# lpastura/kubernetes-1

Measured on AMD Instinct MI355X. Metric: pods scheduled/sec, higher is better.
Workload: dtype int64; 1 GPU; (b) 5000 nodes / 1913000 pods; nodes=5000, nodes_per_gpu=5000, pods=1913000, percentage_of_nodes_to_score=100, parallelism=1 GPU

## Files before the change

include/kgpu.h:

```cpp
#ifndef KGPU_H
#define KGPU_H

#include <stdint.h>

#ifdef __cplusplus
extern "C" {
#endif

#define KGPU_ABI_VERSION 3

#define KGPU_OK 0
#define KGPU_E_INVAL (-1)
#define KGPU_E_NOMEM (-2)
#define KGPU_E_DEVICE (-3)
#define KGPU_E_CAPACITY (-4)
#define KGPU_E_STATE (-5)
#define KGPU_E_UNSUPPORTED (-6)

#define KGPU_CODE_SUCCESS 0
#define KGPU_CODE_ERROR 1
#define KGPU_CODE_UNSCHEDULABLE 2
#define KGPU_CODE_UNRESOLVABLE 3

#define KGPU_F_NODE_UNSCHEDULABLE 0
// ... 383 lines not shown
#define KGPU_OPT_PERSISTENT 2
#define KGPU_OPT_PERSIST_GROUPS 3
#define KGPU_OPT_PHASE_TRACE 4
#define KGPU_OPT_TOPO_FUSED 5
#define KGPU_OPT_TOPO_PERSISTENT 6
#define KGPU_OPT_ABORT_AT 7
#define KGPU_OPT_XGMI 8
#define KGPU_OPT_SKIP_RELEASE_AT 9
#define KGPU_OPT_COOPERATIVE 10
#define KGPU_OPT_BATCH_GEO 11
#define KGPU_OPT_ARENA_BYTES 12
#define KGPU_OPT_TOPO_RESIDENT 13
#define KGPU_OPT_BATCH_HELPER 14
#define KGPU_OPT_TOPO_AHEAD 15
#define KGPU_OPT_TBATCH_GEO 16
#define KGPU_OPT_HOLD_GROUP 17
#define KGPU_OPT_TBATCH_WLAB 18
#define KGPU_OPT_RUN_ALL_FILTERS 20
#define KGPU_OPT_TBATCH_POLL_SLEEP 21
#define KGPU_OPT_ZEROCOPY_POOLS 23
#define KGPU_OPT_CUT_PERSISTENT 24
#define KGPU_OPT_CUT_TOPO_PERSISTENT 25
#define KGPU_OPT_NORM_PERSISTENT 26
int kgpu_set_option(kgpu_ctx* ctx, int32_t option, int64_t value);
int kgpu_debug_counters(const kgpu_ctx* ctx, int64_t* out, int32_t n);
int kgpu_geometry_for(int32_t kernel, int32_t n_nodes, int32_t max_groups, int32_t first, int32_t out[4]);
int kgpu_debug_geometry(const kgpu_ctx* ctx, int32_t out[6]);
int kgpu_debug_instantiation(const kgpu_ctx* ctx, int32_t out[4]);
int kgpu_debug_topo_resident(const kgpu_ctx* ctx, int64_t out[2]);
int kgpu_read_phase_trace(kgpu_ctx* ctx, int64_t* out, int32_t max_iters);

typedef struct kgpu_nominated {
  int32_t node;
  int32_t item;
} kgpu_nominated;
int kgpu_set_nominated(kgpu_ctx* ctx, const kgpu_nominated* noms, int32_t n, const kgpu_pod_query* pods,
                       const kgpu_pools* pools);

typedef struct kgpu_victim {
  int32_t node;
  int32_t slot;
  int32_t item;
  int32_t pad;
  int64_t start_time;
  uint64_t pdb_mask;
} kgpu_victim;
// ... 56 lines not shown
```

kubernetes-1_amd/csrc/kgpu_api.cpp:

```cpp
#include <hip/hip_runtime.h>
#include <rccl/rccl.h>
#include <dlfcn.h>
#include <execinfo.h>
#include <fcntl.h>
#include <signal.h>
#include <unistd.h>

#include <algorithm>
#include <array>
#include <chrono>
#include <atomic>
#include <exception>
#include <memory>
#include <new>
#include <iterator>
#include <cmath>
#include <cstdio>
#include <cstdlib>
#include <cstddef>
#include <cstring>
#include <deque>
#include <map>
#include <string>
#include <unordered_map>
// ... 139 lines not shown
  void* res_pin = nullptr;
  kgpu_result* res_dev = nullptr;
  void* pool_pin = nullptr;
  const char* pool_pin_dev = nullptr;
  bool zc_pools = true;
  kgpu::Arena ar;
  bool tb_abort_mapped = false;
  struct TCache {
    bool valid = false;
    std::string key;
    DevBuf buf[2];
    size_t dirty[2] = {0, 0};
    int cur = 0;
  } tc;
  uint64_t tc_hits = 0, tc_misses = 0;
  bool htrace = false;
  static constexpr int kHt = 18;
  int64_t ht_last = 0, ht_cur[kHt] = {}, ht_n = 0;
  int ht_seen = 0;
  std::vector<std::array<int64_t, kHt>> ht_cycles;
  std::vector<std::array<int64_t, kHt>> ht_batches;
  bool tc_on = true;
  bool batch_helper = true;
  bool topo_ahead = true;
  int tbatch_geo_first = 1;
  size_t ar_limit = 1 << 20;
  DevState ds_last{};
  const void* ds_ptr = nullptr;
  bool last_diag = false;
  std::vector<int64_t> trace_wg_host;
  int32_t trace_wg_groups = 0;
  std::vector<hipEvent_t> ev_pool;
  std::map<std::vector<int64_t>, int> class_ids, tclass_ids;
  std::vector<kgpu::ClassRec> classes;
  std::vector<kgpu::ClassItem> citems;
  std::vector<kgpu::TermClassRec> tclasses;
  std::vector<kgpu_req> creqs;
  std::vector<int32_t> cints;
  int classes_init = 0;
  int Ccap = 0, TCcap = 0;
  DevBuf d_classes, d_citems, d_tclasses, d_creqs, d_cints, d_plans, d_aux, d_aux_terms, scratch, d_pods;
  struct PodRow {
    int32_t node, ns;
    uint32_t flags;
    std::vector<int32_t> pairs;
    std::vector<int32_t> own_tcls;
// ... 2040 lines not shown
      if (cut) {
        const size_t cells = (size_t)cnt * 2 * (size_t)groups;
        const size_t gbytes = (sizeof(uint64_t) * (cells + (size_t)cnt) + 15) & ~(size_t)15;
        if ((rc = ensure(c, c->cgran, gbytes))) return rc;
        HIP_OK(c, hipMemsetAsync(c->cgran.p, 0, gbytes, c->stream));
        ba.cgran = static_cast<uint64_t*>(c->cgran.p);
        ba.cpos = ba.cgran + cells;
        ba.cut_nofilt = c->cfg.n_filters == 0 ? 1 : 0;
        ba.nranks = 1;
        ba.GT = groups;
      } else if (xg) {
        const size_t cells = (size_t)kgpu::kXgmiRing * (size_t)c->xg_GT;
        ba.gran = static_cast<uint64_t*>(c->xg_box.p);
        ba.feas = reinterpret_cast<int32_t*>(ba.gran + cells);
        ba.pgran = static_cast<uint64_t* const*>(c->xg_arr.p);
        ba.pfeas = reinterpret_cast<int32_t* const*>(static_cast<uint64_t* const*>(c->xg_arr.p) + c->xg_nranks);
        ba.nranks = c->xg_nranks;
        ba.rank = c->xg_rank;
        ba.GT = c->xg_GT;
        ba.R = kgpu::kXgmiRing;
        ba.xseq0 = c->xg_seq;
        c->xg_seq += cnt;
      } else {
        const size_t cells = (size_t)cnt * (size_t)groups;
        const size_t gbytes = sizeof(uint64_t) * cells + sizeof(int32_t) * cells;
        if ((rc = ensure(c, c->gran, gbytes))) return rc;
        HIP_OK(c, hipMemsetAsync(c->gran.p, 0, sizeof(uint64_t) * cells, c->stream));
        ba.gran = static_cast<uint64_t*>(c->gran.p);
        ba.feas = reinterpret_cast<int32_t*>(ba.gran + cells);
        run_ptrs.push_back({ba.gran, ba.feas});
        void** slot = static_cast<void**>(c->batch_ptrs.p) + 2 * (run_ptrs.size() - 1);
        if ((rc = stage_h2d(c, slot, run_ptrs.back().data(), sizeof(void*) * 2))) return rc;
        ba.pgran = reinterpret_cast<uint64_t* const*>(slot);
        ba.pfeas = reinterpret_cast<int32_t* const*>(slot + 1);
        ba.nranks = 1;
        ba.rank = 0;
        ba.GT = groups;
        ba.R = 0;
      }
      ba.first = i;
      ba.count = cnt;
      ba.per = per;
      ba.assume = assume;
      ba.seq0 = first_seq + i;
      ba.abort = abort_word;
      ba.abort_at = c->abort_at >= i && c->abort_at < i + cnt ? c->abort_at - i : -1;
      ba.skip_release_at = c->skip_release_at >= i && c->skip_release_at < i + cnt ? c->skip_release_at - i : -1;
// ... 832 lines not shown
  int per = 0, groups = 0;
  const int kidx = kgpu::batch_geometry(c->st.N, std::min(c->max_groups > 0 ? std::min(c->max_groups, c->n_cus) : c->n_cus, 256),
                                        &per, &groups, c->batch_geo_first);
  if (kidx < 0) return fail(c, KGPU_E_UNSUPPORTED, "no persistent geometry for this node count");
  if ((rc = upload_pools(c, pools))) return rc;
  if (!c->ticket.p) {
    if ((rc = ensure(c, c->ticket, 9 * 64))) return rc;
    HIP_OK(c, hipMemset(c->ticket.p, 0, 9 * 64));
  }
  const int s = c->pipe_next;
  c->pipe_next ^= 1;
  kgpu_ctx::PipeSlot& ps = c->pipe[s];
  const size_t q_off = kDsQueryOff, q_bytes = sizeof(kgpu_pod_query) * (size_t)n;
  const size_t p_off = (q_off + q_bytes + 15) & ~(size_t)15, a_off = p_off + 16 * 2;
  const size_t bytes = a_off + 64;
  if ((rc = ensure(c, ps.dev, bytes))) return rc;
  if (ps.host_cap < bytes) {
    if (ps.host) HIP_OK(c, hipHostFree(ps.host));
    ps.host = nullptr;
    ps.host_cap = 0;
    HIP_OK(c, hipHostMalloc(&ps.host, bytes * 2, hipHostMallocDefault));
    ps.host_cap = bytes * 2;
  }
  const size_t cells = (size_t)n * (size_t)groups;
  const size_t gbytes = (sizeof(uint64_t) + sizeof(int32_t)) * cells;
  if (ps.gran.bytes < gbytes) {
    if ((rc = ensure(c, ps.gran, gbytes))) return rc;
    ps.gran_zeroed = 0;
  }
  if (ps.gran_zeroed < gbytes) {
    HIP_OK(c, hipMemsetAsync(ps.gran.p, 0, ps.gran.bytes, c->stream));
    ps.gran_zeroed = ps.gran.bytes;
  }
  const size_t rbytes = sizeof(kgpu_result) * (size_t)n + 64;
  if (ps.res_cap < rbytes) {
    if (ps.res) HIP_OK(c, hipHostFree(ps.res));
    ps.res = nullptr;
    ps.res_cap = 0;
    HIP_OK(c, hipHostMalloc(&ps.res, rbytes * 2, hipHostMallocCoherent | hipHostMallocMapped));
    HIP_OK(c, hipHostGetDevicePointer(&ps.res_dev, ps.res, 0));
    ps.res_cap = rbytes * 2;
  }
  for (hipEvent_t* e : {&ps.done, &ps.t0, &ps.t1})
    if (!*e) HIP_OK(c, hipEventCreateWithFlags(e, e == &ps.done ? hipEventDisableTiming : hipEventDefault));
  char* h = static_cast<char*>(ps.host);
  char* d = static_cast<char*>(ps.dev.p);
  DevState st = c->st;
// ... 1 lines not shown
  st.queries = reinterpret_cast<const kgpu_pod_query*>(d + q_off);
  if ((rc = ensure(c, c->results, sizeof(kgpu_result) * (size_t)n))) return rc;
  st.results = static_cast<kgpu_result*>(c->results.p);
  st.diag_raw = nullptr;
  st.diag_norm = nullptr;
  uint64_t* gran = static_cast<uint64_t*>(ps.gran.p);
  int32_t* feas = reinterpret_cast<int32_t*>(gran + cells);
  std::memcpy(h, &st, sizeof(DevState));
  std::memcpy(h + q_off, qs, q_bytes);
  void* ptrs[2] = {gran, feas};
  std::memcpy(h + p_off, ptrs, sizeof(ptrs));
  std::memset(h + a_off, 0, 64);
  HIP_OK(c, hipMemcpyAsync(d, h, bytes, hipMemcpyHostToDevice, c->stream));
  c->tc.valid = false;
  kgpu::BatchArgs ba{};
  ba.gran = gran;
  ba.feas = feas;
  ba.pgran = reinterpret_cast<uint64_t* const*>(d + p_off);
  ba.pfeas = reinterpret_cast<int32_t* const*>(d + p_off + sizeof(void*));
  ba.nranks = 1;
  ba.rank = 0;
  ba.GT = groups;
  ba.R = 0;
  ba.first = 0;
  ba.count = n;
  ba.per = per;
  ba.assume = 1;
  ba.seq0 = first_seq;
  ba.abort = reinterpret_cast<int32_t*>(d + a_off);
  ba.abort_at = -1;
  ba.skip_release_at = -1;
  ba.trace = nullptr;
  ba.res_out = static_cast<kgpu_result*>(ps.res_dev);
  ba.abort_out = reinterpret_cast<int32_t*>(static_cast<char*>(ps.res_dev) + sizeof(kgpu_result) * (size_t)n);
  kgpu_ctx::PipeSlot& po = c->pipe[s ^ 1];
  ba.zero_buf = static_cast<uint64_t*>(po.gran.p);
  ba.zero_n16 = po.gran.p ? (int64_t)(po.gran.bytes / 16) : 0;
  const bool coop = c->coop;
  ba.hold = -1;
  ++c->n_persist;
  c->n_coop += coop ? 1 : 0;
  *reinterpret_cast<int32_t*>(static_cast<char*>(ps.res) + sizeof(kgpu_result) * (size_t)n) = -1;
  const bool timed = stats != nullptr;
  if (timed) HIP_OK(c, hipEventRecord(ps.t0, c->stream));
  note_geometry(c, 1, kidx, groups, per);
  note_instantiation(c, kgpu::batch_row(c->spec), false, kgpu::batch_helper_used(c->spec, kidx, false, c->batch_helper), n);
// ... 172 lines not shown
      if (cfg->filters[j] == cfg->filters[i]) return KGPU_E_INVAL;
  }
  if (cfg->percentage_of_nodes_to_score < 0 || cfg->percentage_of_nodes_to_score > 100) return KGPU_E_INVAL;
  for (int i = 0; i < cfg->n_scores; ++i)
    if (cfg->scores[i] == KGPU_S_REQUESTED_TO_CAPACITY_RATIO) {
      if (cfg->n_rtcr < 0 || cfg->n_rtcr > 8 || cfg->n_shape < 1 || cfg->n_shape > 16) return KGPU_E_INVAL;
      for (int j = 1; j < cfg->n_shape; ++j)
        if (cfg->shape[j].utilization <= cfg->shape[j - 1].utilization) return KGPU_E_INVAL;
    }
  fail_point();
  std::unique_ptr<kgpu_ctx> holder(new kgpu_ctx());
  kgpu_ctx* c = holder.get();
  int ndev = 0;
  if (hipGetDeviceCount(&ndev) != hipSuccess || ndev <= 0) return KGPU_E_DEVICE;
  if (cfg->device < 0 || cfg->device >= ndev) return KGPU_E_INVAL;
  c->cfg = *cfg;
  c->device = cfg->device;
  if (hipSetDevice(c->device) != hipSuccess) return KGPU_E_DEVICE;
  {
    const char* e = std::getenv("KGPU_SYNC_SPIN");
    if (e && e[0] == '1') (void)hipSetDeviceFlags(hipDeviceScheduleSpin);
  }
  if (const char* e = std::getenv("KGPU_HOST_TRACE")) c->htrace = e[0] == '1';
  if (hipStreamCreateWithFlags(&c->stream, hipStreamNonBlocking) != hipSuccess)
    return KGPU_E_DEVICE;
  hipDeviceProp_t prop;
  if (hipGetDeviceProperties(&prop, c->device) != hipSuccess) {
    (void)hipStreamDestroy(c->stream);
    return KGPU_E_DEVICE;
  }
  c->n_cus = prop.multiProcessorCount;
  DevState& st = c->st;
  st.n_filters = cfg->n_filters;
  std::memcpy(st.filters, cfg->filters, sizeof(st.filters));
  st.n_scores = cfg->n_scores;
  std::memcpy(st.scores, cfg->scores, sizeof(st.scores));
  for (int i = 0; i < KGPU_NUM_SCORES; ++i) st.weights[i] = std::max<int64_t>(cfg->score_weights[i], 1);
  for (int i = 0; i < KGPU_NUM_SCORES; ++i) st.w_of[i] = 0;
  for (int i = 0; i < cfg->n_scores; ++i) st.w_of[cfg->scores[i]] = st.weights[i];
  st.n_least = cfg->n_least;
  st.n_most = cfg->n_most;
  std::memcpy(st.least, cfg->least, sizeof(st.least));
  std::memcpy(st.most, cfg->most, sizeof(st.most));
  st.least_wsum = st.most_wsum = 0;
  for (int i = 0; i < cfg->n_least; ++i) st.least_wsum += cfg->least[i].weight;
  for (int i = 0; i < cfg->n_most; ++i) st.most_wsum += cfg->most[i].weight;
// ... 183 lines not shown
  std::memcpy(out, c->trace_wg_host.data(), sizeof(int64_t) * n);
  *groups = c->trace_wg_groups;
  return (int)std::min<size_t>(n, INT32_MAX);
} catch (...) {
  return on_exception(c, false);
}

int kgpu_set_option(kgpu_ctx* c, int32_t option, int64_t value) try {
  if (c && !c->pipe_q.empty())
    return fail(c, KGPU_E_STATE, "pipelined batches in flight: complete them with kgpu_schedule_batch_wait first");
  if (!c) return KGPU_E_INVAL;
  if (option == KGPU_OPT_KERNEL_TIMING) c->timing = value != 0;
  else if (option == KGPU_OPT_PERSISTENT) c->persistent = value != 0;
  else if (option == KGPU_OPT_PERSIST_GROUPS) c->max_groups = (int)std::max<int64_t>(value, 0);
  else if (option == KGPU_OPT_PHASE_TRACE) {
    c->phase_trace = value != 0;
    c->phase_trace_mode = (int)std::min<int64_t>(std::max<int64_t>(value, 0), 3);
  }
  else if (option == KGPU_OPT_TOPO_FUSED) c->topo_fused = value != 0;
  else if (option == KGPU_OPT_TOPO_PERSISTENT) c->tfast = value != 0;
  else if (option == KGPU_OPT_COOPERATIVE) c->coop = value != 0;
  else if (option == KGPU_OPT_BATCH_GEO) c->batch_geo_first = (int)std::min<int64_t>(std::max<int64_t>(0, value), 6);
  else if (option == KGPU_OPT_BATCH_HELPER) c->batch_helper = value != 0;
  else if (option == KGPU_OPT_TOPO_AHEAD) c->topo_ahead = value != 0;
  else if (option == KGPU_OPT_TBATCH_GEO) c->tbatch_geo_first = (int)std::min<int64_t>(std::max<int64_t>(value, 0), 4);
  else if (option == KGPU_OPT_TOPO_RESIDENT) {
    c->tc_on = value != 0;
    c->tc.valid = false;
  } else if (option == KGPU_OPT_ARENA_BYTES) c->ar_limit = (size_t)std::min<int64_t>(std::max<int64_t>(0, value), (int64_t)kArenaBytes);
  else if (option == KGPU_OPT_ABORT_AT) c->abort_at = value < 0 || value > INT32_MAX ? -1 : (int32_t)value;
  else if (option == KGPU_OPT_XGMI) c->xgmi = value != 0;
  else if (option == KGPU_OPT_TBATCH_WLAB) c->tbatch_wlab = value != 0;
  else if (option == KGPU_OPT_TBATCH_POLL_SLEEP) c->tbatch_sleep = value != 0;
  else if (option == KGPU_OPT_ZEROCOPY_POOLS) c->zc_pools = value != 0;
  else if (option == KGPU_OPT_RUN_ALL_FILTERS) c->run_all = value != 0;
  else if (option == KGPU_OPT_HOLD_GROUP) c->hold_group = value < 0 || value > INT32_MAX ? -1 : (int32_t)value;
  else if (option == KGPU_OPT_CUT_PERSISTENT) c->cut_persistent = value != 0;
  else if (option == KGPU_OPT_CUT_TOPO_PERSISTENT) c->cut_topo_persistent = value != 0;
  else if (option == KGPU_OPT_NORM_PERSISTENT) c->norm_persistent = (int32_t)std::min<int64_t>(std::max<int64_t>(value, 0), INT32_MAX);
  else if (option == KGPU_OPT_SKIP_RELEASE_AT) c->skip_release_at = value < 0 || value > INT32_MAX ? -1 : (int32_t)value;
  else return KGPU_E_INVAL;
  return KGPU_OK;
} catch (...) {
  return on_exception(c, false);
}

// ... 1055 lines not shown
```

kubernetes-1_amd/csrc/kgpu_internal.h:

```cpp
#pragma once
#include <stdint.h>

#include "../../include/kgpu.h"

namespace kgpu {

constexpr int kBlock = 64;
constexpr int kMaxBlocks = 1024;
constexpr int kSelAnd = 0, kSelNothing = 1, kSelEmpty = 2;
constexpr uint64_t kMask40 = (1ull << 40) - 1;
constexpr int kMaxRanks = 64;

struct BlkStat {
  int32_t feasible;
  int32_t max_taint;
  int32_t max_na;
  int32_t pad;
};
struct BlkKey {
  uint64_t key;
  int32_t idx;
  int32_t feasible;
};

// ... 173 lines not shown
  int32_t diag;
  int32_t cut;
  int32_t zero_diag;
  int32_t resolve_self;
  int32_t q_inline;
  int64_t seq;
  int32_t* done_out;
  kgpu_pod_query q;
};

struct BatchArgs {
  int32_t first;
  int32_t count;
  int32_t per;
  int32_t assume;
  int64_t seq0;
  uint64_t* gran;
  int32_t* feas;
  int32_t* abort;
  int64_t* trace;
  int32_t abort_at;
  int32_t skip_release_at;
  int32_t hold;
  int32_t pad_h;
  kgpu_result* res_out;
  int32_t* abort_out;
  uint64_t* zero_buf;
  int64_t zero_n16;
  uint64_t* const* pgran;
  int32_t* const* pfeas;
  int32_t nranks, rank;
  int32_t GT;
  int32_t R;
  int64_t xseq0;
  uint64_t* cgran;
  uint64_t* cpos;
  int32_t cut_nofilt;
  int32_t pad_c;
};
constexpr int32_t kAbortDirty = 1, kAbortClean = 2;
constexpr int kXgmiRing = 4096;
constexpr int kXgmiMaxGT = 1024;

constexpr int kTMaxSoftWords = 8;
constexpr int kTMaxZones = 32;
constexpr int kTLdsBudget = 144 * 1024;
constexpr int kTCutBytes = 544;
// ... 241 lines not shown
```

kubernetes-1_amd/csrc/kgpu_kernels.hip:

```cpp
#include <hip/hip_runtime.h>

#include <algorithm>
#include <map>
#include <mutex>
#include <tuple>
#include <type_traits>

#include "kgpu_internal.h"

#if defined(__HIP_DEVICE_COMPILE__)
#define GAS __attribute__((address_space(1)))
#define CAS __attribute__((address_space(4)))
#else
#define GAS
#define CAS
#endif

namespace kgpu {

template <class T>
__device__ __forceinline__ GAS T* gp(T* p) {
  return (GAS T*)p;
}
template <class T>
// ... 1302 lines not shown
  }
  if (!__all(all)) return false;
  wave_argmax(k, gsel);
  wkey = k;
  wg = k ? gsel : -1;
  return true;
}
template <int NJ, bool SYS>
__device__ __forceinline__ bool poll_row(const uint64_t* row, int G, const int32_t* abort_word, uint64_t tmask,
                                         uint64_t expect, uint64_t& wkey, int& wg) {
  const uint64_t t0 = __builtin_amdgcn_s_memrealtime();
  Sweep<NJ> a = sweep<NJ, SYS>(row, G, abort_word, expect);
  for (;;) {
    const Sweep<NJ> b = sweep<NJ, SYS>(row, G, abort_word, expect);
    if (a.abort != 0) return false;
    if (row_done<NJ>(a, tmask, expect, wkey, wg)) return true;
    a = sweep<NJ, SYS>(row, G, abort_word, expect);
    if (b.abort != 0) return false;
    if (row_done<NJ>(b, tmask, expect, wkey, wg)) return true;
    if (__builtin_amdgcn_s_memrealtime() - t0 > kSpinTimeout) return false;
  }
}

struct HRow {
  int64_t ac, am, zc, zm;
  double ic, im;
};

constexpr int kQRing = 4;
constexpr int kQWords = (int)(sizeof(kgpu_pod_query) / 8);
static_assert(kQWords <= 64, "one query row per vector load");
typedef uint64_t __attribute__((may_alias)) qword_t;
struct NoQuery {};
__device__ __forceinline__ kgpu_pod_query ring_read(const kgpu_pod_query* ring, int k) {
  const kgpu_pod_query& s = ring[k & (kQRing - 1)];
  kgpu_pod_query q{};
  q.flags = s.flags;
  q.req[0] = s.req[0]; q.req[1] = s.req[1]; q.req[2] = s.req[2];
  q.nz[0] = s.nz[0]; q.nz[1] = s.nz[1];
  q.score_req[0] = s.score_req[0]; q.score_req[1] = s.score_req[1];
  q.scalars = s.scalars;
  q.ports = s.ports;
  return q;
}
__device__ __forceinline__ kgpu_pod_query ring_uniform(kgpu_pod_query q) {
  q.flags = __builtin_amdgcn_readfirstlane(q.flags);
  q.scalars.begin = __builtin_amdgcn_readfirstlane(q.scalars.begin);
  q.scalars.count = __builtin_amdgcn_readfirstlane(q.scalars.count);
  q.ports.begin = __builtin_amdgcn_readfirstlane(q.ports.begin);
  q.ports.count = __builtin_amdgcn_readfirstlane(q.ports.count);
  return q;
}

template <uint32_t FM, uint32_t SM, int K, int B, bool XG, bool HB = false, bool TR = false>
__global__ __launch_bounds__(B + 64 + (HB ? 2 * B : 0)) void k_batch(const DevState* __restrict__ stp, BatchArgs pa) {
  static_assert(!HB || (B == 64 && !XG &&
                       SM == ((1u << KGPU_S_BALANCED_ALLOCATION) | (1u << KGPU_S_LEAST_ALLOCATED) | kDefRes)),
                "the helper wave splits config (b)'s profile on the one-row-wave geometry");
  static_assert(HB || !TR, "only the helper-wave instantiation has a traced twin");
  const DevState& st = *stp;
  constexpr int W = B / 64;
  const int tid = threadIdx.x, wave = tid >> 6, lane = tid & 63;
  const int G = gridDim.x, g = blockIdx.x;
  if (g == pa.hold) return;
  const int lo = g * pa.per;
  const int GT = pa.GT, gme = pa.rank * G + g;
  constexpr bool xg = XG;
  const uint64_t tmask = xg ? (0xFull << 60) : kGValid;
  __shared__ BatchShared<B> sh;
  __shared__ int64_t sh_hk[HB ? 2 * 2 * K * B : 1];
  __shared__ int sh_hready[2];
  __shared__ std::conditional_t<HB, kgpu_pod_query, NoQuery> sh_q[HB ? kQRing : 1];
  __shared__ uint64_t* sh_peer_g[XG ? kMaxRanks : 1];
  __shared__ int32_t* sh_peer_f[XG ? kMaxRanks : 1];
  if constexpr (XG) {
    if (wave == W && lane < pa.nranks) {
      sh_peer_g[lane] = pa.pgran[lane];
      sh_peer_f[lane] = pa.pfeas[lane];
    }
  }
  if (tid == 0) {
    sh.bready = 0;
// ... 4 lines not shown
  if constexpr (HB) {
    if (wave == W && lane < kQWords)
      for (int k = 0; k < 3 && k < pa.count; ++k)
        reinterpret_cast<qword_t*>(&sh_q[k])[lane] = ((const GAS qword_t*)(st.queries + pa.first + k))[lane];
  }
  __syncthreads();
  auto ring_row = [&](int k) -> size_t { return xg ? (size_t)((pa.xseq0 + k) % pa.R) : (size_t)k; };
  auto ring_tag = [&](int k) -> uint64_t {
    return xg ? (kGValid | ((uint64_t)(((pa.xseq0 + k) / pa.R) & 7) << 60)) : kGValid;
  };
  auto publish = [&](int i, uint64_t key, int feas) {
    const size_t roff = ring_row(i) * GT + gme;
    const uint64_t gtag = ring_tag(i);
    if constexpr (!XG) {
      store_sc1(pa.gran + roff, gtag | key);
      pa.feas[roff] = feas;
    } else {
      for (int rk = 0; rk < pa.nranks; ++rk) {
        __hip_atomic_store(sh_peer_g[rk] + roff, gtag | key, __ATOMIC_RELAXED, __HIP_MEMORY_SCOPE_SYSTEM);
        __hip_atomic_store(sh_peer_f[rk] + roff, feas, __ATOMIC_RELAXED, __HIP_MEMORY_SCOPE_SYSTEM);
      }
    }
  };
  const bool tr = pa.trace && (g == 0 || g == G - 1);
  int64_t* trow = pa.trace ? pa.trace + (g == 0 ? 0 : 8) : nullptr;
  constexpr bool kStamps = !HB || TR;
#define KGPU_STAMP(i, k) \
  if (kStamps && tr && (tid == 0 || tid == B)) trow[(size_t)(i) * 16 + (k)] = (int64_t)__builtin_amdgcn_s_memrealtime()

  if constexpr (HB) {
    if (wave == W + 1 || wave == W + 2) {
      const int hw = wave - W - 1;
      HRow h[K];
#pragma unroll
      for (int j = 0; j < K; ++j) {
        const int n = lo + j * B + lane;
        h[j] = HRow{0, 0, 0, 0, 0.0, 0.0};
        if (!spare_slot(j, K, lane, B) && n < st.N) {
          h[j].ac = gp(st.alloc_cpu)[n];
          h[j].am = gp(st.alloc_mem)[n];
          h[j].zc = gp(st.nz_cpu)[n];
          h[j].zm = gp(st.nz_mem)[n];
          h[j].ic = (h[j].ac > 0 && h[j].ac < (1ll << 52)) ? 1.0 / (double)h[j].ac : 0.0;
          h[j].im = (h[j].am > 0 && h[j].am < (1ll << 52)) ? 1.0 / (double)h[j].am : 0.0;
        }
      }
// ... 55 lines not shown
        }
        rqp = rq;
        rq = ring_uniform(rqn);
        const bool slow = have_cur && won && pa.assume && !fast_b;
        int cn = -1;
        if (have_cur && !slow) {
          const Cand c = wg_combine<B>(sh, p, won && fast_b);
          cn = c.key ? c.idx : -1;
        }
        if (slow) {
          lds_wait(&sh.cready, i + 1, pa.abort);
          cand = sh.cslow[p];
        } else {
          cand = cn;
        }
        staged = have_cur && !slow && cand >= 0;
      }
      return;
    }
  }
  if (wave == W) {
    int cand = -1;
    bool staged = false;
    for (int i = 0; i <= pa.count; ++i) {
      const bool have_prev = i > 0, have_cur = i < pa.count;
      const int p = i & 1;
      if (i == pa.abort_at && g == 0 && lane == 0) __hip_atomic_store(pa.abort, 1, __ATOMIC_RELAXED, __HIP_MEMORY_SCOPE_AGENT);
      uint64_t qv = 0;
      if constexpr (HB) {
        if (i + 3 < pa.count && lane < kQWords) qv = ((const GAS qword_t*)(st.queries + pa.first + i + 3))[lane];
      } else if (i + 2 < pa.count) {
        const uint64_t v = lane < kQWords ? reinterpret_cast<const uint64_t*>(st.queries + pa.first + i + 2)[lane] : 0;
        asm volatile("" ::"v"(v));
      }
      bool qmem = false;
      if (have_prev) {
        if constexpr (HB) {
          const kgpu_pod_query& qq = sh_q[(i - 1) & (kQRing - 1)];
          qmem = __builtin_amdgcn_readfirstlane(qq.scalars.count | qq.ports.count) != 0;
        } else {
          const kgpu_pod_query* qq = st.queries + pa.first + i - 1;
          qmem = (cp(qq)->scalars.count | cp(qq)->ports.count) != 0;
        }
      }
      const bool fast_b = have_prev && cand >= 0 && staged && pa.assume && !qmem;
      uint64_t wkey = 0;
      int wg = -1;
      bool ok = true;
      if (have_prev) {
        const uint64_t* prow = pa.gran + ring_row(i - 1) * GT;
        const uint64_t expect = ring_tag(i - 1);
        if constexpr (!XG)
          ok = poll_row<4, false>(prow, GT, pa.abort, tmask, expect, wkey, wg);
        else if (GT <= 256)
          ok = poll_row<4, true>(prow, GT, pa.abort, tmask, expect, wkey, wg);
        else
          ok = poll_row<16, true>(prow, GT, pa.abort, tmask, expect, wkey, wg);
        KGPU_STAMP(i, 7);
      }
      const bool won = have_prev && wg == gme;
      const bool slow = have_cur && won && pa.assume && !fast_b;
      if (ok) {
        if (have_prev && lane == 0 && (xg ? g == 0 : (won || (wg < 0 && g == 0)))) {
          kgpu_result res;
          res.node = wg < 0 ? -1
                   : xg ? (int32_t)rank40_inv(pod_tie_key(st.seed, pa.seq0 + i - 1), wkey & kMask40, st.tie_mode)
                        : st.node_base + lo + cand;
          res.feasible = 0;
          res.evaluated = st.n_total;
          res.scored = 0;
          res.score = wg >= 0 ? (int64_t)(wkey >> 40) - 1 : 0;
          gp(st.results)[pa.first + i - 1] = res;
        }
      } else if (lane == 0) {
        __hip_atomic_fetch_or(pa.abort, (i <= 1 && !XG) ? kAbortClean : kAbortDirty, __ATOMIC_RELAXED,
                              __HIP_MEMORY_SCOPE_AGENT);
      }
      if (lane == 0 && have_prev) {
        sh.rwg[(i - 1) & 1] = wg;
        sh.rabort[(i - 1) & 1] = ok ? 0 : 1;
      }
      __syncthreads();
      if (!ok) break;
      int cn = -1;
      if (have_cur && !slow) {
        KGPU_STAMP(i, 6);
        const Cand c = wg_combine<B>(sh, p, won && fast_b);
        if (lane == 0) publish(i, c.key, c.feas);
        KGPU_STAMP(i, 3);
        cn = c.key ? c.idx : -1;
      }
      if constexpr (HB) {
        if (i + 3 < pa.count && lane < kQWords) reinterpret_cast<qword_t*>(&sh_q[(i + 3) & (kQRing - 1)])[lane] = qv;
      }
      if (slow) {
        lds_wait(&sh.cready, i + 1, pa.abort);
        cand = sh.cslow[p];
      } else {
        cand = cn;
      }
      staged = have_cur && !slow && cand >= 0;
    }
    return;
  }

  constexpr bool kStream = K > 4;
  constexpr int KR = kStream ? 1 : K;
  static_assert(!kStream || (W > 1 && !HB), "streamed rows: the candidate row travels through sh.brow");
  constexpr bool kRecip = (SM & kDefRes) != 0 && SM != kRuntime;
  NodeRes r[KR];
#pragma unroll
  for (int j = 0; j < KR; ++j) {
    const int n = lo + j * B + tid;
    r[j] = NodeRes{};
    if (!kStream && !spare_slot(j, K, tid, B) && n < st.N) r[j] = load_row<kRecip>(st, n);
  }
  __builtin_amdgcn_s_waitcnt(0);

  kgpu_pod_query qp{};
  kgpu_pod_query q = *cp(st.queries + pa.first);
  if constexpr (HB) q = ring_uniform(ring_read(sh_q, 0));
  int cand = -1;
  bool staged = false;
  for (int i = 0; i <= pa.count; ++i) {
    KGPU_STAMP(i, 0);
    std::conditional_t<HB, kgpu_pod_query, NoQuery> qraw{};
    if constexpr (HB) qraw = ring_read(sh_q, i + 1);
    const bool have_prev = i > 0;
    const bool have_cur = i < pa.count;
    const int p = i & 1;
    const bool fast_b = have_prev && cand >= 0 && staged && pa.assume && qp.scalars.count == 0 && qp.ports.count == 0;
    const int ob = cand >= 0 ? cand % B : -1, jb = cand >= 0 ? cand / B : -1;
    uint64_t keys[K];
    Cand own_a{0, -1, 0}, own_b{0, -1, 0};
    if (have_cur) {
      const uint64_t tk = pod_tie_key(st.seed, pa.seq0 + i);
      if (fast_b && wave == W - 1) {
        NodeRes t;
        if constexpr (W == 1) {
#pragma unroll
          for (int j = 0; j < K; ++j)
            if (j == jb) t = lane_row(r[j], ob);
        } else {
          lds_wait(&sh.bready, i, pa.abort);
          t = sh.brow[(i - 1) & 1];
        }
        assume_regs(qp, t);
        if (tid == B - 1) r[KR - 1] = t;
      }
      if constexpr (HB) {
        uint32_t fs[K];
        uint64_t rkj[K];
#pragma unroll
        for (int j = 0; j < K; ++j) {
          const bool spare = spare_slot(j, K, tid, B);
          const int n = spare ? lo + cand : lo + j * B + tid;
          fs[j] = (spare ? fast_b : n < st.N) ? run_filters<FM>(st, q, r[j], n) : 1u;
// ... 4 lines not shown
        lds_wait_ge(&sh_hready[1], i + 1, pa.abort);
#pragma unroll
        for (int j = 0; j < K; ++j) {
          const int64_t tot = sh_hk[((0 * 2 + p) * K + j) * B + tid] + sh_hk[((1 * 2 + p) * K + j) * B + tid];
          keys[j] = fs[j] ? 0 : (((uint64_t)(tot + 1) << 40) | rkj[j]);
        }
      } else {
#pragma unroll
        for (int j = 0; j < K; ++j) {
          const bool spare = spare_slot(j, K, tid, B);
          const int n = spare ? lo + cand : lo + j * B + tid;
          if constexpr (kStream) {
            const bool live = spare ? fast_b : n < st.N;
            NodeRes rj = r[0];
            if (!spare && live) rj = load_row<kRecip>(st, n);
            keys[j] = live ? node_key<FM, SM>(st, q, rj, n, tk) : 0;
          } else {
            keys[j] = (spare ? fast_b : n < st.N) ? node_key<FM, SM>(st, q, r[j], n, tk) : 0;
          }
        }
      }
      KGPU_STAMP(i, 5);
      wg_partials<K, B>(sh, p, keys, fast_b, ob, jb, cand, own_a, own_b);
    }
    KGPU_STAMP(i, 1);
    kgpu_pod_query qn{};
    if constexpr (!HB) {
      if (i + 1 < pa.count) qn = *cp(st.queries + pa.first + i + 1);
    }
    __syncthreads();
    KGPU_STAMP(i, 2);
    int wg = -1;
    if (have_prev) {
      const int s = (i - 1) & 1;
      if (sh.rabort[s]) break;
      wg = sh.rwg[s];
    }
    if constexpr (HB) {
      if (i + 1 < pa.count) qn = ring_uniform(qraw);
    }
    const bool won = have_prev && wg == gme;
    int cn = -1;
    if (have_cur) {
      if (won && pa.assume && !fast_b) {
        cn = -2;
      } else {
// ... 8 lines not shown
          if constexpr (kStream) {
            NodeRes t = load_res(st, lo + (j * B + tid));
            assume_row(st, qp, t, lo + (j * B + tid));
          } else {
            assume_row(st, qp, r[j], lo + (j * B + tid));
          }
          assume_counts(st, pa.first + i - 1, lo + (j * B + tid));
        }
    }
    const bool slow = cn == -2;
    if (slow) {
      if (wave == ob / 64) {
        if (tid == ob) {
          const uint64_t tk = pod_tie_key(st.seed, pa.seq0 + i);
#pragma unroll
          for (int j = 0; j < K; ++j)
            if (j == jb) {
              if constexpr (kStream) keys[j] = node_key<FM, SM>(st, q, load_row<kRecip>(st, lo + (j * B + tid)), lo + (j * B + tid), tk);
              else keys[j] = node_key<FM, SM>(st, q, r[j], lo + (j * B + tid), tk);
            }
        }
        const Cand c = wave_recombine<K, B>(sh, p, keys);
        if (lane == 0) {
          publish(i, c.key, c.feas);
          sh.cslow[p] = c.key ? c.idx : -1;
          lds_release(&sh.cready, i + 1);
        }
      }
      lds_wait(&sh.cready, i + 1, pa.abort);
      cand = sh.cslow[p];
    } else {
      cand = cn;
      if (W > 1 && cand >= 0 && tid == cand % B) {
#pragma unroll
        for (int j = 0; j < K; ++j)
          if (j == cand / B) {
            if constexpr (kStream) sh.brow[p] = load_row<kRecip>(st, lo + cand);
            else sh.brow[p] = r[j];
          }
        if (i != pa.skip_release_at) lds_release(&sh.bready, i + 1);
      }
    }
    staged = have_cur && !slow && cand >= 0;
    qp = q;
    q = qn;
    KGPU_STAMP(i, 4);
  }
#undef KGPU_STAMP
}

__global__ __launch_bounds__(256) void k_batch_fixup(const DevState* __restrict__ stp, BatchArgs pa, int G) {
  const DevState& st = *stp;
  const int lane = threadIdx.x & 63;
  const int i = blockIdx.x * 4 + (threadIdx.x >> 6);
  for (int64_t z = (int64_t)blockIdx.x * blockDim.x + threadIdx.x; z < pa.zero_n16; z += (int64_t)gridDim.x * blockDim.x) {
    uint4* zp = reinterpret_cast<uint4*>(pa.zero_buf) + z;
    *zp = uint4{0, 0, 0, 0};
  }
  if (pa.abort_out && blockIdx.x == 0 && threadIdx.x == 0)
    __hip_atomic_store(pa.abort_out, load_sc1(pa.abort), __ATOMIC_RELAXED, __HIP_MEMORY_SCOPE_SYSTEM);
  if (i >= pa.count) return;
  const size_t row = pa.R > 0 ? (size_t)((pa.xseq0 + i) % pa.R) : (size_t)i;
  int f = 0;
  for (int g = lane; g < pa.GT; g += 64) f += pa.feas[row * pa.GT + g];
  f = (int)wave_sum32((uint32_t)f);
  (void)G;
  if (lane == 0) {
    kgpu_result& r = gp(st.results)[pa.first + i];
    r.feasible = f;
    if (r.node >= 0 && f >= 2) {
      r.scored = 1;
    } else {
      r.scored = 0;
      r.score = 0;
    }
    if (pa.res_out) pa.res_out[pa.first + i] = r;
  }
}

template <int NJ>
__device__ __forceinline__ bool poll_counts(const uint64_t* row, int G, int g, const int32_t* abort_word,
                                            uint32_t (&out)[4]) {
  const int lane = threadIdx.x & 63;
  const uint64_t t0 = __builtin_amdgcn_s_memrealtime();
  for (;;) {
    const Sweep<NJ> a = sweep<NJ, false>(row, G, abort_word, kGValid);
    if (__any(a.abort != 0)) return false;
// ... 2731 lines not shown

struct Geo {
  int B, K;
};
constexpr Geo kGeo[] = {{64, 1}, {128, 1}, {192, 1}, {448, 1}, {960, 1}, {512, 4}, {512, 8}};
constexpr int kNumGeo = sizeof(kGeo) / sizeof(kGeo[0]);
constexpr int kBatchLdsPad = 96 * 1024;

template <uint32_t FM, uint32_t SM>
struct BatchRow {
  using Fn = void (*)(const DevState*, BatchArgs);
  static constexpr Fn fn[kNumGeo] = {k_batch<FM, SM, 1, 64, false>,  k_batch<FM, SM, 1, 128, false>,
                                     k_batch<FM, SM, 1, 192, false>, k_batch<FM, SM, 1, 448, false>,
                                     k_batch<FM, SM, 1, 960, false>, k_batch<FM, SM, 4, 512, false>,
                                     k_batch<FM, SM, 8, 512, false>};
  static constexpr Fn xfn[kNumGeo] = {k_batch<FM, SM, 1, 64, true>,  k_batch<FM, SM, 1, 128, true>,
                                      k_batch<FM, SM, 1, 192, true>, k_batch<FM, SM, 1, 448, true>,
                                      k_batch<FM, SM, 1, 960, true>, k_batch<FM, SM, 4, 512, true>,
                                      k_batch<FM, SM, 8, 512, true>};
};
using BatchFn = void (*)(const DevState*, BatchArgs);
template <uint32_t FM, uint32_t SM, bool E>
struct HelperFn {
  static constexpr BatchFn fn = nullptr, traced = nullptr;
};
template <uint32_t FM, uint32_t SM>
struct HelperFn<FM, SM, true> {
  static constexpr BatchFn fn = k_batch<FM, SM, 1, 64, false, true>;
  static constexpr BatchFn traced = k_batch<FM, SM, 1, 64, false, true, true>;
};
static const BatchFn kBatchHelper[] = {
    nullptr,
    HelperFn<kFitFM, kFitSM, true>::fn,
    nullptr,
    nullptr,
};
static const BatchFn kBatchHelperTraced[] = {
    nullptr,
    HelperFn<kFitFM, kFitSM, true>::traced,
    nullptr,
    nullptr,
};
static const BatchFn* const kBatch[] = {
    BatchRow<kRuntime, kRuntime>::fn,
    BatchRow<kFitFM, kFitSM>::fn,
    BatchRow<kDefaultFM, kDefaultSM>::fn,
    BatchRow<kDefaultFM, kAutoscalerSM>::fn,
};
static_assert(sizeof(kBatch) / sizeof(kBatch[0]) == kNumSpecs, "one k_batch row per profile instantiation");
static const BatchFn* const kBatchX[] = {
    BatchRow<kRuntime, kRuntime>::xfn,
    BatchRow<kFitFM, kFitSM>::xfn,
    BatchRow<kDefaultFM, kDefaultSM>::xfn,
    BatchRow<kDefaultFM, kAutoscalerSM>::xfn,
};

int batch_geometry(int N, int max_groups, int* per, int* groups, int first) {
  for (int gi = first < 0 ? 0 : first; gi < kNumGeo; ++gi) {
    const int p = kGeo[gi].B * kGeo[gi].K - 1;
    const int g = (N + p - 1) / p;
    if (g <= max_groups) {
      *per = p;
// ... 11 lines not shown
    return true;
  }
  if (kernel == 2 && geo >= 0 && geo < kNumTGeo) {
    *threads = kTGeo[geo].B;
    *rows = kTGeo[geo].K;
    return true;
  }
  return false;
}

int batch_row(int spec) { return spec < 0 || spec >= kNumSpecs ? 0 : spec; }

bool batch_helper_used(int spec, int geo, bool sharded, bool helper) {
  return helper && !sharded && geo == 0 && kBatchHelper[batch_row(spec)] != nullptr;
}

int launch_batch(const DevState* st, const BatchArgs& a, int groups, int geo, int spec, bool coop, bool helper,
                 void* stream) {
  spec = batch_row(spec);
  if (geo < 0 || geo >= kNumGeo) return -1;
  const int x = a.R > 0 ? 1 : 0;
  const bool hb = batch_helper_used(spec, geo, x != 0, helper);
  const bool traced = hb && a.trace != nullptr;
  const BatchFn fn = hb ? (traced ? kBatchHelperTraced : kBatchHelper)[spec] : (x ? kBatchX : kBatch)[spec][geo];
  const int threads = kGeo[geo].B + 64 + (hb ? 2 * kGeo[geo].B : 0);
  static bool attr_set[4][kNumSpecs][kNumGeo] = {};
  const int ai = hb ? (traced ? 3 : 2) : x;
  if (!attr_set[ai][spec][geo]) {
    if (hipFuncSetAttribute(reinterpret_cast<const void*>(fn), hipFuncAttributeMaxDynamicSharedMemorySize,
                            kBatchLdsPad) != hipSuccess)
      return -1;
    attr_set[ai][spec][geo] = true;
  }
  BatchArgs arg = a;
  const DevState* sp = st;
  void* args[] = {(void*)&sp, (void*)&arg};
  if (!coop && grid_fits(reinterpret_cast<const void*>(fn), threads, (size_t)kBatchLdsPad, groups)) {
    hipLaunchKernelGGL(fn, dim3(groups), dim3(threads), (unsigned)kBatchLdsPad, (hipStream_t)stream, sp, arg);
    if (hipGetLastError() != hipSuccess) return -1;
  } else {
    arg.hold = -1;
    if (hipLaunchCooperativeKernel(reinterpret_cast<const void*>(fn), dim3(groups), dim3(threads), args,
                                   (unsigned)kBatchLdsPad, (hipStream_t)stream) != hipSuccess)
      return -1;
  }
  hipLaunchKernelGGL(k_batch_fixup, dim3((a.count + 3) / 4), dim3(256), 0, (hipStream_t)stream, st, a, groups);
  return hipGetLastError() == hipSuccess ? 0 : -1;
}

template <uint32_t FM, uint32_t SM>
// ... 679 lines not shown
```

kubernetes-1_amd/kgpu/abi.py:

```python
import ctypes as C

import numpy as np

ABI_VERSION = 3
OK, E_INVAL, E_NOMEM, E_DEVICE, E_CAPACITY, E_STATE, E_UNSUPPORTED = 0, -1, -2, -3, -4, -5, -6
ERRNAMES = {0: "OK", -1: "KGPU_E_INVAL", -2: "KGPU_E_NOMEM", -3: "KGPU_E_DEVICE", -4: "KGPU_E_CAPACITY",
            -5: "KGPU_E_STATE", -6: "KGPU_E_UNSUPPORTED"}

OPT_KERNEL_TIMING, OPT_PERSISTENT, OPT_PERSIST_GROUPS, OPT_PHASE_TRACE, OPT_TOPO_FUSED = 1, 2, 3, 4, 5
OPT_TOPO_PERSISTENT = 6
OPT_ABORT_AT = 7
OPT_XGMI = 8
OPT_SKIP_RELEASE_AT = 9
OPT_COOPERATIVE = 10
OPT_BATCH_GEO = 11
OPT_ARENA_BYTES = 12
OPT_TOPO_RESIDENT = 13
OPT_BATCH_HELPER = 14
OPT_TOPO_AHEAD = 15
OPT_TBATCH_GEO = 16
OPT_HOLD_GROUP = 17
OPT_TBATCH_WLAB = 18
OPT_RUN_ALL_FILTERS = 20
OPT_TBATCH_POLL_SLEEP = 21
OPT_ZEROCOPY_POOLS = 23
OPT_CUT_PERSISTENT = 24
OPT_CUT_TOPO_PERSISTENT = 25
OPT_NORM_PERSISTENT = 26
CODE_SUCCESS, CODE_ERROR, CODE_UNSCHEDULABLE, CODE_UNRESOLVABLE = 0, 1, 2, 3
STATUS_NOT_EVALUATED = 0xFF

F_NODE_UNSCHEDULABLE, F_FIT, F_NODE_NAME, F_NODE_PORTS, F_NODE_AFFINITY, F_TAINT, F_PTS, F_IPA = range(8)
NUM_FILTERS = 8
FILTER_IDS = {"NodeUnschedulable": 0, "NodeResourcesFit": 1, "NodeName": 2, "NodePorts": 3, "NodeAffinity": 4,
              "TaintToleration": 5, "PodTopologySpread": 6, "InterPodAffinity": 7}
FILTER_NAMES = {v: k for k, v in FILTER_IDS.items()}

(S_BALANCED, S_IMAGE, S_IPA, S_LEAST, S_NODE_AFFINITY, S_NPAP, S_PTS, S_DPTS, S_TAINT, S_MOST, S_RTCR,
 S_LIMITS) = range(12)
NUM_SCORES = 12
SCORE_IDS = {"NodeResourcesBalancedAllocation": 0, "ImageLocality": 1, "InterPodAffinity": 2,
             "NodeResourcesLeastAllocated": 3, "NodeAffinity": 4, "NodePreferAvoidPods": 5,
             "PodTopologySpread": 6, "DefaultPodTopologySpread": 7, "TaintToleration": 8,
             "NodeResourcesMostAllocated": 9, "RequestedToCapacityRatio": 10, "NodeResourceLimits": 11}
SCORE_NAMES = {v: k for k, v in SCORE_IDS.items()}

OP_IN, OP_NOTIN, OP_EXISTS, OP_DNE, OP_GT, OP_LT = range(6)
SEL_AND, SEL_NOTHING = 0, 1
TERM_REQ_AFF, TERM_REQ_ANTI, TERM_PREF_AFF, TERM_PREF_ANTI = range(4)
PF_TERMINATING, PF_WITH_AFFINITY, PF_ACTIVE = 1, 2, 4
(Q_TOLERATES_UNSCHED, Q_FIT_ALL_ZERO, Q_HAS_TSC, Q_HAS_POD_AFFINITY, Q_HAS_POD_ANTI, Q_SELF_MATCH_ALL_AFF,
# ... 136 lines not shown
```

Baseline: 681,400 pods/s.

## Publish dual speculative per-group candidates early in helper-wave batch kernel

Adds an early-publish mode to the helper-wave batch kernel. Each group publishes two candidate keys per row right after computing partials: one assuming it did not win the previous pod and one assuming it did. The poller picks the right one using the previous winner group. This is meant to take the cross-group wait for the previous row's outcome off the critical path, at the cost of twice the gran/feas buffer size, wider stores and more complex polling.

Measured after the change: 796,000 pods/s (median of 6 runs). 1.17x the previous value.

```diff
diff --git a/include/kgpu.h b/include/kgpu.h
--- a/include/kgpu.h
+++ b/include/kgpu.h
@@ -429,6 +429,7 @@
 #define KGPU_OPT_CUT_PERSISTENT 24
 #define KGPU_OPT_CUT_TOPO_PERSISTENT 25
 #define KGPU_OPT_NORM_PERSISTENT 26
+#define KGPU_OPT_BATCH_EARLY_PUBLISH 27
 int kgpu_set_option(kgpu_ctx* ctx, int32_t option, int64_t value);
 int kgpu_debug_counters(const kgpu_ctx* ctx, int64_t* out, int32_t n);
 int kgpu_geometry_for(int32_t kernel, int32_t n_nodes, int32_t max_groups, int32_t first, int32_t out[4]);
diff --git a/kubernetes-1_amd/csrc/kgpu_api.cpp b/kubernetes-1_amd/csrc/kgpu_api.cpp
--- a/kubernetes-1_amd/csrc/kgpu_api.cpp
+++ b/kubernetes-1_amd/csrc/kgpu_api.cpp
@@ -185,6 +185,7 @@
   std::vector<std::array<int64_t, kHt>> ht_batches;
   bool tc_on = true;
   bool batch_helper = true;
+  bool batch_early = true;
   bool topo_ahead = true;
   int tbatch_geo_first = 1;
   size_t ar_limit = 1 << 20;
@@ -2271,7 +2272,8 @@
         ba.xseq0 = c->xg_seq;
         c->xg_seq += cnt;
       } else {
-        const size_t cells = (size_t)cnt * (size_t)groups;
+        ba.dual = c->batch_early && kgpu::batch_helper_used(c->spec, kidx, false, c->batch_helper) ? 1 : 0;
+        const size_t cells = (size_t)cnt * (size_t)groups * (ba.dual ? 2 : 1);
         const size_t gbytes = sizeof(uint64_t) * cells + sizeof(int32_t) * cells;
         if ((rc = ensure(c, c->gran, gbytes))) return rc;
         HIP_OK(c, hipMemsetAsync(c->gran.p, 0, sizeof(uint64_t) * cells, c->stream));
@@ -3150,7 +3152,8 @@
     HIP_OK(c, hipHostMalloc(&ps.host, bytes * 2, hipHostMallocDefault));
     ps.host_cap = bytes * 2;
   }
-  const size_t cells = (size_t)n * (size_t)groups;
+  const bool dual = c->batch_early && kgpu::batch_helper_used(c->spec, kidx, false, c->batch_helper);
+  const size_t cells = (size_t)n * (size_t)groups * (dual ? 2 : 1);
   const size_t gbytes = (sizeof(uint64_t) + sizeof(int32_t)) * cells;
   if (ps.gran.bytes < gbytes) {
     if ((rc = ensure(c, ps.gran, gbytes))) return rc;
@@ -3198,6 +3201,7 @@
   ba.rank = 0;
   ba.GT = groups;
   ba.R = 0;
+  ba.dual = dual ? 1 : 0;
   ba.first = 0;
   ba.count = n;
   ba.per = per;
@@ -3416,6 +3420,7 @@
     if (e && e[0] == '1') (void)hipSetDeviceFlags(hipDeviceScheduleSpin);
   }
   if (const char* e = std::getenv("KGPU_HOST_TRACE")) c->htrace = e[0] == '1';
+  if (const char* e = std::getenv("KGPU_BATCH_EARLY_PUBLISH")) c->batch_early = e[0] != '0';
   if (hipStreamCreateWithFlags(&c->stream, hipStreamNonBlocking) != hipSuccess)
     return KGPU_E_DEVICE;
   hipDeviceProp_t prop;
@@ -3645,6 +3650,7 @@
   else if (option == KGPU_OPT_COOPERATIVE) c->coop = value != 0;
   else if (option == KGPU_OPT_BATCH_GEO) c->batch_geo_first = (int)std::min<int64_t>(std::max<int64_t>(0, value), 6);
   else if (option == KGPU_OPT_BATCH_HELPER) c->batch_helper = value != 0;
+  else if (option == KGPU_OPT_BATCH_EARLY_PUBLISH) c->batch_early = value != 0;
   else if (option == KGPU_OPT_TOPO_AHEAD) c->topo_ahead = value != 0;
   else if (option == KGPU_OPT_TBATCH_GEO) c->tbatch_geo_first = (int)std::min<int64_t>(std::max<int64_t>(value, 0), 4);
   else if (option == KGPU_OPT_TOPO_RESIDENT) {
diff --git a/kubernetes-1_amd/csrc/kgpu_internal.h b/kubernetes-1_amd/csrc/kgpu_internal.h
--- a/kubernetes-1_amd/csrc/kgpu_internal.h
+++ b/kubernetes-1_amd/csrc/kgpu_internal.h
@@ -219,7 +219,7 @@
   int32_t abort_at;
   int32_t skip_release_at;
   int32_t hold;
-  int32_t pad_h;
+  int32_t dual;
   kgpu_result* res_out;
   int32_t* abort_out;
   uint64_t* zero_buf;
diff --git a/kubernetes-1_amd/csrc/kgpu_kernels.hip b/kubernetes-1_amd/csrc/kgpu_kernels.hip
--- a/kubernetes-1_amd/csrc/kgpu_kernels.hip
+++ b/kubernetes-1_amd/csrc/kgpu_kernels.hip
@@ -1348,6 +1348,65 @@
   }
 }
 
+template <int NJ>
+struct Sweep2 {
+  uint64_t a[NJ], b[NJ];
+  int abort;
+};
+template <int NJ>
+__device__ __forceinline__ Sweep2<NJ> sweep2(const uint64_t* row, int G, const int32_t* abort_word, uint64_t fill) {
+  const int lane = threadIdx.x & 63;
+  Sweep2<NJ> s;
+#pragma unroll
+  for (int j = 0; j < NJ; ++j) {
+    const uint64_t* p = row + 2 * (lane + 64 * j);
+    const bool in = lane + 64 * j < G;
+    s.a[j] = in ? load_sc1(p) : fill;
+    s.b[j] = in ? load_sc1(p + 1) : fill;
+  }
+  s.abort = load_sc1(abort_word);
+  return s;
+}
+template <int NJ>
+__device__ __forceinline__ bool row_done2(const Sweep2<NJ>& cur, int wb, uint64_t& wkey, int& wg) {
+  const int lane = threadIdx.x & 63;
+  bool all = true;
+  uint64_t k = 0;
+  int gsel = -1;
+#pragma unroll
+  for (int j = 0; j < NJ; ++j) {
+    if (!(cur.a[j] & cur.b[j] & kGValid)) {
+      all = false;
+    } else {
+      const uint64_t v = (lane + 64 * j == wb ? cur.b[j] : cur.a[j]) & ~kGValid;
+      if (v > k) {
+        k = v;
+        gsel = lane + 64 * j;
+      }
+    }
+  }
+  if (!__all(all)) return false;
+  wave_argmax(k, gsel);
+  wkey = k;
+  wg = k ? gsel : -1;
+  return true;
+}
+template <int NJ>
+__device__ __forceinline__ bool poll_row2(const uint64_t* row, int G, const int32_t* abort_word, int wb, uint64_t& wkey,
+                                          int& wg) {
+  const uint64_t t0 = __builtin_amdgcn_s_memrealtime();
+  Sweep2<NJ> a = sweep2<NJ>(row, G, abort_word, kGValid);
+  for (;;) {
+    const Sweep2<NJ> b = sweep2<NJ>(row, G, abort_word, kGValid);
+    if (a.abort != 0) return false;
+    if (row_done2<NJ>(a, wb, wkey, wg)) return true;
+    a = sweep2<NJ>(row, G, abort_word, kGValid);
+    if (b.abort != 0) return false;
+    if (row_done2<NJ>(b, wb, wkey, wg)) return true;
+    if (__builtin_amdgcn_s_memrealtime() - t0 > kSpinTimeout) return false;
+  }
+}
+
 struct HRow {
   int64_t ac, am, zc, zm;
   double ic, im;
@@ -1378,12 +1437,13 @@
   return q;
 }
 
-template <uint32_t FM, uint32_t SM, int K, int B, bool XG, bool HB = false, bool TR = false>
+template <uint32_t FM, uint32_t SM, int K, int B, bool XG, bool HB = false, bool TR = false, bool EP = false>
 __global__ __launch_bounds__(B + 64 + (HB ? 2 * B : 0)) void k_batch(const DevState* __restrict__ stp, BatchArgs pa) {
   static_assert(!HB || (B == 64 && !XG &&
                        SM == ((1u << KGPU_S_BALANCED_ALLOCATION) | (1u << KGPU_S_LEAST_ALLOCATED) | kDefRes)),
                 "the helper wave splits config (b)'s profile on the one-row-wave geometry");
   static_assert(HB || !TR, "only the helper-wave instantiation has a traced twin");
+  static_assert(HB || !EP, "only the helper-wave instantiation publishes early");
   const DevState& st = *stp;
   constexpr int W = B / 64;
   const int tid = threadIdx.x, wave = tid >> 6, lane = tid & 63;
@@ -1434,6 +1494,15 @@
       }
     }
   };
+  auto publish2 = [&](int i, uint64_t ka, uint64_t kb, int fa, int fb) {
+    const size_t roff = (size_t)i * GT + gme;
+    typedef uint32_t __attribute__((ext_vector_type(4))) u32x4;
+    const uint64_t wa = kGValid | ka, wb = kGValid | kb;
+    const u32x4 v = {(uint32_t)wa, (uint32_t)(wa >> 32), (uint32_t)wb, (uint32_t)(wb >> 32)};
+    GAS uint64_t* gp2 = (GAS uint64_t*)(pa.gran + 2 * roff);
+    asm volatile("global_store_dwordx4 %0, %1, off sc1\n\ts_nop 1" ::"v"(gp2), "v"(v) : "memory");
+    reinterpret_cast<int2*>(pa.feas)[roff] = int2{fa, fb};
+  };
   const bool tr = pa.trace && (g == 0 || g == G - 1);
   int64_t* trow = pa.trace ? pa.trace + (g == 0 ? 0 : 8) : nullptr;
   constexpr bool kStamps = !HB || TR;
@@ -1535,6 +1604,7 @@
   if (wave == W) {
     int cand = -1;
     bool staged = false;
+    int wprev = -1;
     for (int i = 0; i <= pa.count; ++i) {
       const bool have_prev = i > 0, have_cur = i < pa.count;
       const int p = i & 1;
@@ -1563,7 +1633,10 @@
       if (have_prev) {
         const uint64_t* prow = pa.gran + ring_row(i - 1) * GT;
         const uint64_t expect = ring_tag(i - 1);
-        if constexpr (!XG)
+        if constexpr (EP)
+          ok = GT <= 128 ? poll_row2<2>(pa.gran + (size_t)(i - 1) * 2 * GT, GT, pa.abort, wprev, wkey, wg)
+                         : poll_row2<4>(pa.gran + (size_t)(i - 1) * 2 * GT, GT, pa.abort, wprev, wkey, wg);
+        else if constexpr (!XG)
           ok = poll_row<4, false>(prow, GT, pa.abort, tmask, expect, wkey, wg);
         else if (GT <= 256)
           ok = poll_row<4, true>(prow, GT, pa.abort, tmask, expect, wkey, wg);
@@ -1571,6 +1644,7 @@
           ok = poll_row<16, true>(prow, GT, pa.abort, tmask, expect, wkey, wg);
         KGPU_STAMP(i, 7);
       }
+      wprev = wg;
       const bool won = have_prev && wg == gme;
       const bool slow = have_cur && won && pa.assume && !fast_b;
       if (ok) {
@@ -1597,10 +1671,12 @@
       if (!ok) break;
       int cn = -1;
       if (have_cur && !slow) {
-        KGPU_STAMP(i, 6);
+        if constexpr (!EP) KGPU_STAMP(i, 6);
         const Cand c = wg_combine<B>(sh, p, won && fast_b);
-        if (lane == 0) publish(i, c.key, c.feas);
-        KGPU_STAMP(i, 3);
+        if constexpr (!EP) {
+          if (lane == 0) publish(i, c.key, c.feas);
+          KGPU_STAMP(i, 3);
+        }
         cn = c.key ? c.idx : -1;
       }
       if constexpr (HB) {
@@ -1646,6 +1722,7 @@
     const int ob = cand >= 0 ? cand % B : -1, jb = cand >= 0 ? cand / B : -1;
     uint64_t keys[K];
     Cand own_a{0, -1, 0}, own_b{0, -1, 0};
+    bool defer = false;
     if (have_cur) {
       const uint64_t tk = pod_tie_key(st.seed, pa.seq0 + i);
       if (fast_b && wave == W - 1) {
@@ -1696,6 +1773,15 @@
       }
       KGPU_STAMP(i, 5);
       wg_partials<K, B>(sh, p, keys, fast_b, ob, jb, cand, own_a, own_b);
+      if constexpr (EP) {
+        defer = have_prev && cand >= 0 && pa.assume && !fast_b;
+        KGPU_STAMP(i, 6);
+        if (!defer) {
+          if (lane == 0)
+            publish2(i, own_a.key, fast_b ? own_b.key : own_a.key, own_a.feas, fast_b ? own_b.feas : own_a.feas);
+          KGPU_STAMP(i, 3);
+        }
+      }
     }
     KGPU_STAMP(i, 1);
     kgpu_pod_query qn{};
@@ -1750,7 +1836,8 @@
         }
         const Cand c = wave_recombine<K, B>(sh, p, keys);
         if (lane == 0) {
-          publish(i, c.key, c.feas);
+          if constexpr (EP) publish2(i, c.key, c.key, c.feas, c.feas);
+          else publish(i, c.key, c.feas);
           sh.cslow[p] = c.key ? c.idx : -1;
           lds_release(&sh.cready, i + 1);
         }
@@ -1758,6 +1845,12 @@
       lds_wait(&sh.cready, i + 1, pa.abort);
       cand = sh.cslow[p];
     } else {
+      if constexpr (EP) {
+        if (have_cur && defer) {
+          if (lane == 0) publish2(i, own_a.key, own_a.key, own_a.feas, own_a.feas);
+          KGPU_STAMP(i, 3);
+        }
+      }
       cand = cn;
       if (W > 1 && cand >= 0 && tid == cand % B) {
 #pragma unroll
@@ -1790,7 +1883,16 @@
   if (i >= pa.count) return;
   const size_t row = pa.R > 0 ? (size_t)((pa.xseq0 + i) % pa.R) : (size_t)i;
   int f = 0;
-  for (int g = lane; g < pa.GT; g += 64) f += pa.feas[row * pa.GT + g];
+  if (pa.dual) {
+    int wb = -1;
+    if (i > 0) {
+      const int pn = gp(st.results)[pa.first + i - 1].node;
+      if (pn >= 0) wb = (pn - st.node_base) / pa.per;
+    }
+    for (int g = lane; g < pa.GT; g += 64) f += pa.feas[(row * pa.GT + g) * 2 + (g == wb ? 1 : 0)];
+  } else {
+    for (int g = lane; g < pa.GT; g += 64) f += pa.feas[row * pa.GT + g];
+  }
   f = (int)wave_sum32((uint32_t)f);
   (void)G;
   if (lane == 0) {
@@ -4568,12 +4670,14 @@
 using BatchFn = void (*)(const DevState*, BatchArgs);
 template <uint32_t FM, uint32_t SM, bool E>
 struct HelperFn {
-  static constexpr BatchFn fn = nullptr, traced = nullptr;
+  static constexpr BatchFn fn = nullptr, traced = nullptr, early = nullptr, early_traced = nullptr;
 };
 template <uint32_t FM, uint32_t SM>
 struct HelperFn<FM, SM, true> {
   static constexpr BatchFn fn = k_batch<FM, SM, 1, 64, false, true>;
   static constexpr BatchFn traced = k_batch<FM, SM, 1, 64, false, true, true>;
+  static constexpr BatchFn early = k_batch<FM, SM, 1, 64, false, true, false, true>;
+  static constexpr BatchFn early_traced = k_batch<FM, SM, 1, 64, false, true, true, true>;
 };
 static const BatchFn kBatchHelper[] = {
     nullptr,
@@ -4584,6 +4688,18 @@
 static const BatchFn kBatchHelperTraced[] = {
     nullptr,
     HelperFn<kFitFM, kFitSM, true>::traced,
+    nullptr,
+    nullptr,
+};
+static const BatchFn kBatchHelperEarly[] = {
+    nullptr,
+    HelperFn<kFitFM, kFitSM, true>::early,
+    nullptr,
+    nullptr,
+};
+static const BatchFn kBatchHelperEarlyTraced[] = {
+    nullptr,
+    HelperFn<kFitFM, kFitSM, true>::early_traced,
     nullptr,
     nullptr,
 };
@@ -4641,10 +4757,14 @@
   const int x = a.R > 0 ? 1 : 0;
   const bool hb = batch_helper_used(spec, geo, x != 0, helper);
   const bool traced = hb && a.trace != nullptr;
-  const BatchFn fn = hb ? (traced ? kBatchHelperTraced : kBatchHelper)[spec] : (x ? kBatchX : kBatch)[spec][geo];
+  const bool early = a.dual != 0;
+  if (early && !hb) return -1;
+  const BatchFn fn = hb ? (early ? (traced ? kBatchHelperEarlyTraced : kBatchHelperEarly)
+                                 : (traced ? kBatchHelperTraced : kBatchHelper))[spec]
+                        : (x ? kBatchX : kBatch)[spec][geo];
   const int threads = kGeo[geo].B + 64 + (hb ? 2 * kGeo[geo].B : 0);
-  static bool attr_set[4][kNumSpecs][kNumGeo] = {};
-  const int ai = hb ? (traced ? 3 : 2) : x;
+  static bool attr_set[6][kNumSpecs][kNumGeo] = {};
+  const int ai = hb ? (traced ? 3 : 2) + (early ? 2 : 0) : x;
   if (!attr_set[ai][spec][geo]) {
     if (hipFuncSetAttribute(reinterpret_cast<const void*>(fn), hipFuncAttributeMaxDynamicSharedMemorySize,
                             kBatchLdsPad) != hipSuccess)
diff --git a/kubernetes-1_amd/kgpu/abi.py b/kubernetes-1_amd/kgpu/abi.py
--- a/kubernetes-1_amd/kgpu/abi.py
+++ b/kubernetes-1_amd/kgpu/abi.py
@@ -27,6 +27,7 @@
 OPT_CUT_PERSISTENT = 24
 OPT_CUT_TOPO_PERSISTENT = 25
 OPT_NORM_PERSISTENT = 26
+OPT_BATCH_EARLY_PUBLISH = 27
 CODE_SUCCESS, CODE_ERROR, CODE_UNSCHEDULABLE, CODE_UNRESOLVABLE = 0, 1, 2, 3
 STATUS_NOT_EVALUATED = 0xFF
 
```
